# heng-hw/SpaCap3D

Measured on AMD Instinct MI355X. Metric: scenes/sec (40k pts, 256 proposals) fwd+bwd, higher is better.
Workload: dtype f32; 1 GPU; cfg2: synthetic ScanRefer-shaped scans, 40000 pts x (xyz+1 ch), 256 proposals, 8 scenes/GPU; full training step (SpaCapNet fwd + loss + bwd + grad all-reduce + Adam); global_batch=8, parallelism=dp1, hip_graph=True, fps_prefetch_side_stream=True, prefetch_as_graph=True, reserved_cus_forward=8, geometry_prefetch=True, deferred_weight_gradients=True, params=9290918, allreduce_bytes=35572416

## Files before the change

spacap3d_amd/csrc/sa_mlp.hip:

```cpp
#include <hipcub/hipcub.hpp>

#include <type_traits>

#include "common.hpp"
#include "mfma.hpp"
#include <atomic>

namespace {
using namespace spacap::mfma;

constexpr int TM = 64;
constexpr int TW = 32;
constexpr int NPART = 1024;


__device__ __forceinline__ long row_div(long r, long d) {
  if (((unsigned long long)r | (unsigned long long)d) >> 32) return r / d;
  return (long)((unsigned)r / (unsigned)d);
}

__device__ __forceinline__ f32x4 l1_row(f32x4 wx, f32x4 wy, f32x4 wz, f32x4 wf, f32x4 in, bool has_feat) {
  f32x4 z = wx * in[0] + wy * in[1] + wz * in[2];
  if (has_feat) z += wf * in[3];
  return z;
// ... 337 lines not shown
#pragma unroll
        for (int q = 0; q < KH; ++q)
#pragma unroll
          for (int u = 0; u < 4; ++u)
#pragma unroll
            for (int j = 0; j < NT; ++j)
              acc[mt][j] = MFMA16(wf[j][(h * KH + q) * 4 + u], bq[c & 1][q][u], acc[mt][j]);
        __builtin_amdgcn_sched_barrier(0);
        if (c + 2 < NCH) bload(c + 2);
      }
    }
#pragma unroll
    for (int mt = 0; mt < TMT / 16; ++mt)
#pragma unroll
      for (int j = 0; j < NT; ++j) {
        if (TAIL) {
          f32x4 v = acc[mt][j] + bv[j];
#pragma unroll
          for (int u = 0; u < 4; ++u) v[u] = fmaxf(v[u], 0.f);
          st4(&s_o[(mt * 16 + l15) * LDO + wc + 16 * j + 4 * lg], v);
        } else {
          st4(&s_o[(mt * 16 + l15) * LDO + wc + 16 * j + 4 * lg], acc[mt][j]);
          if (FULL || row0 + mt * 16 + l15 < R) {
            ssum[j] += acc[mt][j];
            ssq[j] += acc[mt][j] * acc[mt][j];
          }
        }
      }
    __syncthreads();
#pragma unroll
    for (int i = 0; i < NO; ++i) {
      const int row = or0 + i * OSTEP;
      if (FULL || row0 + row < R) st4(zout + (size_t)(row0 + row) * Cout + cbb + o4 * 4, ld4(&s_o[row * LDO + o4 * 4]));
    }
    if (TAIL) {
      f32x4 a3 = {0.f, 0.f, 0.f, 0.f};
#pragma unroll
      for (int ks = 0; ks < COB / 4; ++ks) a3 = MFMA16(wf3[TAIL ? ks : 0], s_o[(w * 16 + l15) * LDO + ks * 4 + lg], a3);
      const long row = row0 + w * 16 + l15;
      if (FULL || row < R) {
#pragma unroll
        for (int u = 0; u < 4; ++u)
          if (4 * lg + u < ta.NO3) ta.pred[(size_t)row * ta.NO3 + 4 * lg + u] = a3[u] + ta.b3[4 * lg + u];
      }
    }
  };
  const long nfull = R / TMT;
  bool pending = false;
  if ((long)blockIdx.x < nfull) fetch(blockIdx.x);
  for (long t = blockIdx.x; t < nfull; t += gridDim.x) {
    tile(t, std::true_type{}, pending);
    pending = true;
  }
  asm volatile("s_waitcnt vmcnt(0)" ::: "memory");
#pragma unroll
  for (int i = 0; i < NV; ++i) asm volatile("" ::"v"(pre[i]));
  if (nfull < ntiles && (long)blockIdx.x == nfull % gridDim.x) {
    fetch(nfull);
    tile(nfull, std::false_type{}, false);
  }
  if (TAIL) return;
#pragma unroll
  for (int j = 0; j < NT; ++j)
#pragma unroll
    for (int u = 0; u < 4; ++u) {
      float a = ssum[j][u], q = ssq[j][u];
#pragma unroll
      for (int o = 1; o < 16; o <<= 1) a += __shfl_xor(a, o), q += __shfl_xor(q, o);
      if (l15 == 0) {
        const int c = cb + 16 * j + 4 * lg + u;
        part[((size_t)blockIdx.x * 2 + 0) * Cout + c] = (double)a;
        part[((size_t)blockIdx.x * 2 + 1) * Cout + c] = (double)q;
        for (int pr = blockIdx.x + gridDim.x; pr < NPART; pr += gridDim.x)
          part[((size_t)pr * 2 + 0) * Cout + c] = 0.0, part[((size_t)pr * 2 + 1) * Cout + c] = 0.0;
      }
    }
}

using f32x16 = float __attribute__((ext_vector_type(16)));
#define MFMA_BF16(a, b, c) __builtin_amdgcn_mfma_f32_32x32x16_bf16((a), (b), (c), 0, 0, 0)

#include "sa_bf3.inc"
#include "sa_bf3_dgrad.inc"
#include "sa_l3bwd.inc"

__global__ __launch_bounds__(256) void sa_pool_fwd_kernel(const float *__restrict__ z, const float *__restrict__ st,
                                                          long G, int S, int C, float *__restrict__ out,
                                                          uint8_t *__restrict__ arg) {
  const int C4 = C / 4;
  const long i = (long)blockIdx.x * 256 + threadIdx.x;
  if (i >= G * C4) return;
  const long g = i / C4;
  const int c4 = (int)(i % C4);
  f32x4 mean, sc, be;
#pragma unroll
  for (int u = 0; u < 4; ++u) {
    const float *s = st + (size_t)(c4 * 4 + u) * 4;
    mean[u] = s[0], sc[u] = s[2], be[u] = s[3];
  }
  f32x4 best = {-1.f, -1.f, -1.f, -1.f};
  int bi[4] = {0, 0, 0, 0};
  const float *p = z + ((size_t)g * S) * C + c4 * 4;
#pragma unroll 4
  for (int s = 0; s < S; ++s, p += C) {
    const f32x4 v = ld4(p);
#pragma unroll
    for (int u = 0; u < 4; ++u) {
      const float a = fmaxf((v[u] - mean[u]) * sc[u] + be[u], 0.f);
      if (a > best[u]) best[u] = a, bi[u] = s;
    }
  }
  st4(out + (size_t)g * C + c4 * 4, best);
  *reinterpret_cast<uchar4 *>(arg + (size_t)g * C + c4 * 4) =
      make_uchar4((unsigned char)bi[0], (unsigned char)bi[1], (unsigned char)bi[2], (unsigned char)bi[3]);
}

__global__ __launch_bounds__(256) void sa_pool_bwd_kernel(const float *__restrict__ dout, const float *__restrict__ out,
                                                          const uint8_t *__restrict__ arg, const float *__restrict__ z,
                                                          const float *__restrict__ zmax, const float *__restrict__ st, long G,
                                                          int S, int C, float *__restrict__ dym, double *__restrict__ part) {
  __shared__ float s_red[2][256];
  const int tid = threadIdx.x;
  const int c = tid % C;
  const int gs = tid / C, GP = 256 / C;
  const float mean = st[c * 4], istd = st[c * 4 + 1];
  const bool from_max = zmax && (st[c * 4 + 2] != 0.f || !z);
  float s1 = 0.f, s2 = 0.f;
  for (long g = (long)blockIdx.x * GP + gs; g < G; g += (long)gridDim.x * GP) {
    const size_t o = (size_t)g * C + c;
    const float dy = out[o] > 0.f ? dout[o] : 0.f;
    dym[o] = dy;
    const float zz = from_max ? zmax[o] : z[((size_t)g * S + arg[o]) * C + c];
    s1 += dy;
    s2 += dy * ((zz - mean) * istd);
  }
  s_red[0][tid] = s1, s_red[1][tid] = s2;
  __syncthreads();
  if (tid < C) {
    double a = 0.0, b = 0.0;
    for (int i = 0; i < GP; ++i) a += (double)s_red[0][i * C + tid], b += (double)s_red[1][i * C + tid];
    part[((size_t)blockIdx.x * 2 + 0) * C + tid] = a;
    part[((size_t)blockIdx.x * 2 + 1) * C + tid] = b;
  }
}

template <bool POOLED>
__device__ __forceinline__ f32x4 load_dz(const float *__restrict__ dy, const uint8_t *__restrict__ arg, int S,
                                         const float *__restrict__ zk, long grow, int CK, int c0, f32x4 g, f32x4 k0,
                                         f32x4 k1) {
  const f32x4 z = ld4(zk + (size_t)grow * CK + c0);
  f32x4 d;
  if (POOLED) {
    const int lgS = (S & (S - 1)) == 0 ? __builtin_ctz((unsigned)S) : -1;
    const long grp = lgS >= 0 ? (grow >> lgS) : grow / S;
    const int s = (int)(grow - grp * S);
    const f32x4 dm = ld4(dy + (size_t)grp * CK + c0);
    const uchar4 a = *reinterpret_cast<const uchar4 *>(arg + (size_t)grp * CK + c0);
    d[0] = a.x == s ? dm[0] : 0.f;
    d[1] = a.y == s ? dm[1] : 0.f;
    d[2] = a.z == s ? dm[2] : 0.f;
    d[3] = a.w == s ? dm[3] : 0.f;
  } else {
    d = ld4(dy + (size_t)grow * CK + c0);
  }
  return g * d + k0 - k1 * z;
}

struct L1Args {
  const float *feat, *xyz, *new_xyz;
  const int32_t *idx;
  float rdiv;
  int Np, N, S;
  float *part;
  const float *rel4;
  L1In li;
  float *partW;
};

template <int CK, int NT, bool POOLED, bool PREFETCH, bool ALIAS, bool L1 = false, bool WG = false>
__global__ __launch_bounds__(256) __attribute__((amdgpu_waves_per_eu(L1 ? 2 : 1))) void sa_dgrad_kernel(const float *__restrict__ dy, const uint8_t *__restrict__ arg, int S,
                                                       const float *__restrict__ zk, const float *__restrict__ coef,
                                                       const float *__restrict__ Wk, int CP, const float *__restrict__ zp,
                                                       const float *__restrict__ st_p, long R, float *__restrict__ dyp,
                                                       double *__restrict__ part, const L1Args L = L1Args{}) {
  constexpr int LD = CK + 4, KS = CK / 4, C4 = CK / 4, NV = TM * C4 / 256, RSTEP = 256 / C4;
  constexpr int COB = 64 * NT, LDO = COB + 4, O4 = COB / 4, NO = TM * O4 / 256, OSTEP = 256 / O4;
  constexpr bool DENSE_PF = PREFETCH && !POOLED;
  extern __shared__ __attribute__((aligned(16))) float smem[];
  float *s_a = smem;
  float *s_o = ALIAS ? smem : smem + TM * LD;
  const int tid = threadIdx.x, lane = tid & 63, w = tid >> 6, l15 = lane & 15, lg = lane >> 4;
  const int cbb = blockIdx.y * COB, wc = w * 16 * NT, cb = cbb + wc;
  float wf[NT][KS];
#pragma unroll
  for (int j = 0; j < NT; ++j)
#pragma unroll
    for (int ks = 0; ks < KS; ++ks) wf[j][ks] = Wk[(size_t)(ks * 4 + lg) * CP + cb + 16 * j + l15];
  const int c4 = tid % C4, r0 = tid / C4, o4 = tid % O4, or0 = tid / O4;
  f32x4 g, k0, k1, pm, pi, ps, pb;
#pragma unroll
  for (int u = 0; u < 4; ++u) {
    const float *s = coef + (size_t)(c4 * 4 + u) * 4;
    g[u] = s[0], k0[u] = s[1], k1[u] = s[2];
    const float *q = st_p + (size_t)(cbb + o4 * 4 + u) * 4;
    pm[u] = q[0], pi[u] = q[1], ps[u] = q[2], pb[u] = q[3];
  }
  f32x4 s1 = {0.f, 0.f, 0.f, 0.f}, s2 = {0.f, 0.f, 0.f, 0.f};
  const int lgS = (S > 0 && (S & (S - 1)) == 0) ? __builtin_ctz((unsigned)S) : -1;
  const long ntiles = (R + TM - 1) / TM, nfull = R / TM;
  float *s_rel = smem + (ALIAS ? TM * LD : TM * LD + TM * LDO);
  f32x4 q1[L1 ? 4 : 1], q3[L1 ? 4 : 1], q2 = {0.f, 0.f, 0.f, 0.f};
  f32x4 l1x = {0.f, 0.f, 0.f, 0.f}, l1y = l1x, l1z = l1x, l1f = l1x;
  if (L1 && L.rel4) l1_weights(L.li, cbb + o4 * 4, l1x, l1y, l1z, l1f);
  if (L1) {
#pragma unroll
    for (int u = 0; u < 4; ++u) q1[u] = q3[u] = f32x4{0.f, 0.f, 0.f, 0.f};
  }
  static_assert(!WG || (L1 && !ALIAS && CK == 64 && NT == 1), "fused weight gradient: 64 x 64 first-layer instance only");
  f32x4 accw[WG ? 4 : 1];
#pragma unroll
  for (int n = 0; n < (WG ? 4 : 1); ++n) accw[n] = f32x4{0.f, 0.f, 0.f, 0.f};
  f32x4 pz[PREFETCH ? NV : 1], pd[DENSE_PF ? NV : 1];
  auto fetch = [&](long t) {
#pragma unroll
    for (int i = 0; i < NV; ++i) {
      long grow = t * TM + r0 + i * RSTEP;
      grow = grow < R ? grow : R - 1;
      const float *src = zk + (size_t)grow * CK + c4 * 4;
      asm volatile("global_load_dwordx4 %0, %1, off" : "=&v"(pz[i]) : "v"(src) : "memory");
      if (DENSE_PF) {
        const float *sd = dy + (size_t)grow * CK + c4 * 4;
        asm volatile("global_load_dwordx4 %0, %1, off" : "=&v"(pd[i]) : "v"(sd) : "memory");
      }
    }
  };
  auto tile = [&](long t, auto full, bool stores_pending) {
    constexpr bool FULL = decltype(full)::value;
    const long row0 = t * TM;
    if (PREFETCH) {
      if (stores_pending && !L1) asm volatile("s_waitcnt vmcnt(%0)" ::"n"(NO) : "memory");
      else asm volatile("s_waitcnt vmcnt(0)" ::: "memory");
#pragma unroll
      for (int i = 0; i < NV; ++i) {
        asm volatile("" : "+v"(pz[i]));
        if (DENSE_PF) asm volatile("" : "+v"(pd[i]));
      }
    }
#pragma unroll
    for (int i = 0; i < NV; ++i) {
      const int row = r0 + i * RSTEP;
      const long grow = row0 + row;
      f32x4 a = {0.f, 0.f, 0.f, 0.f};
      if (FULL || grow < R) {
        const f32x4 z = PREFETCH ? pz[i] : ld4(zk + (size_t)grow * CK + c4 * 4);
        f32x4 d;
        if (POOLED) {
          const long grp = lgS >= 0 ? (grow >> lgS) : grow / S;
          const int sidx = (int)(grow - grp * S);
          const f32x4 dm = ld4(dy + (size_t)grp * CK + c4 * 4);
          const uchar4 am = *reinterpret_cast<const uchar4 *>(arg + (size_t)grp * CK + c4 * 4);
          d[0] = am.x == sidx ? dm[0] : 0.f;
          d[1] = am.y == sidx ? dm[1] : 0.f;
          d[2] = am.z == sidx ? dm[2] : 0.f;
          d[3] = am.w == sidx ? dm[3] : 0.f;
        } else {
          d = DENSE_PF ? pd[i] : ld4(dy + (size_t)grow * CK + c4 * 4);
        }
        a = g * d + k0 - k1 * z;
      }
      st4(&s_a[row * LD + c4 * 4], a);
    }
    if (L1 && tid < TM) {
      f32x4 in = {0.f, 0.f, 0.f, 0.f};
      const long grow = row0 + tid;
      if ((FULL || grow < R) && L.rel4) {
        in = ld4(L.rel4 + (size_t)grow * 4);
      } else if (FULL || grow < R) {
        const long b = row_div(grow, (long)L.N * L.S), gi = row_div(grow, L.S);
        const int p = L.idx[grow];
        const float *q = L.xyz + ((size_t)b * L.Np + p) * 3, *c = L.new_xyz + (size_t)gi * 3;
        in[0] = (q[0] - c[0]) / L.rdiv, in[1] = (q[1] - c[1]) / L.rdiv, in[2] = (q[2] - c[2]) / L.rdiv;
        if (L.feat) in[3] = L.feat[(size_t)b * L.Np + p];
      }
      st4(&s_rel[tid * 4], in);
      q2 += in;
    }
    __syncthreads();
    if (PREFETCH && FULL) fetch(t + gridDim.x);
    f32x4 acc[TM / 16][NT];
#pragma unroll
    for (int mt = 0; mt < TM / 16; ++mt)
#pragma unroll
      for (int j = 0; j < NT; ++j) acc[mt][j] = f32x4{0.f, 0.f, 0.f, 0.f};
    {
#pragma unroll
      for (int ks = 0; ks < KS; ++ks) {
#pragma unroll
        for (int mt = 0; mt < TM / 16; ++mt) {
          const float b = s_a[(mt * 16 + l15) * LD + ks * 4 + lg];
#pragma unroll
          for (int j = 0; j < NT; ++j) acc[mt][j] = MFMA16(wf[j][ks], b, acc[mt][j]);
        }
      }
    }
    if (ALIAS) __syncthreads();
#pragma unroll
    for (int mt = 0; mt < TM / 16; ++mt)
#pragma unroll
      for (int j = 0; j < NT; ++j) st4(&s_o[(mt * 16 + l15) * LDO + wc + 16 * j + 4 * lg], acc[mt][j]);
    __syncthreads();
#pragma unroll
    for (int i = 0; i < NO; ++i) {
      const int row = or0 + i * OSTEP;
      if (FULL || row0 + row < R) {
        const size_t o = (size_t)(row0 + row) * CP + cbb + o4 * 4;
        const f32x4 da = ld4(&s_o[row * LDO + o4 * 4]);
        f32x4 z;
        if (L1 && L.rel4) z = l1_row(l1x, l1y, l1z, l1f, ld4(&s_rel[row * 4]), L.li.has_feat != 0);
        else z = ld4(zp + o);
        f32x4 d;
#pragma unroll
        for (int u = 0; u < 4; ++u) {
          const float pre = (z[u] - pm[u]) * ps[u] + pb[u];
          d[u] = pre > 0.f ? da[u] : 0.f;
          s1[u] += d[u];
          s2[u] += d[u] * ((z[u] - pm[u]) * pi[u]);
        }
        if (L1) {
          const f32x4 in = ld4(&s_rel[row * 4]);
#pragma unroll
          for (int u = 0; u < 4; ++u) {
            q1[u] += in * d[u];
            q3[u] += in * z[u];
          }
        } else {
          st4(dyp + o, d);
        }
        if (WG) {
          f32x4 ap;
#pragma unroll
          for (int u = 0; u < 4; ++u) ap[u] = fmaxf((z[u] - pm[u]) * ps[u] + pb[u], 0.f);
          st4(&s_o[row * LDO + o4 * 4], ap);
        }
      } else if (WG) {
        st4(&s_o[row * LDO + o4 * 4], f32x4{0.f, 0.f, 0.f, 0.f});
      }
    }
    if (WG) {
      __syncthreads();
#pragma unroll
      for (int ks = 0; ks < TM / 4; ++ks) {
        const float af = s_a[(ks * 4 + lg) * LD + 16 * w + l15];
#pragma unroll
        for (int n = 0; n < 4; ++n) accw[n] = MFMA16(af, s_o[(ks * 4 + lg) * LDO + 16 * n + l15], accw[n]);
      }
      __syncthreads();
    }
    if (ALIAS) __syncthreads();
  };
  bool pending = false;
  if (PREFETCH && (long)blockIdx.x < nfull) fetch(blockIdx.x);
  for (long t = blockIdx.x; t < nfull; t += gridDim.x) {
    tile(t, std::true_type{}, pending);
    pending = true;
  }
  if (PREFETCH) {
    asm volatile("s_waitcnt vmcnt(0)" ::: "memory");
#pragma unroll
    for (int i = 0; i < NV; ++i) {
      asm volatile("" ::"v"(pz[i]));
      if (DENSE_PF) asm volatile("" ::"v"(pd[i]));
    }
  }
  if (nfull < ntiles && (long)blockIdx.x == nfull % gridDim.x) {
    if (PREFETCH) {
      fetch(nfull);
    }
    tile(nfull, std::false_type{}, false);
  }
  __syncthreads();
  float *s_red = smem;
  st4(&s_red[(0 * OSTEP + or0) * COB + o4 * 4], s1);
  st4(&s_red[(1 * OSTEP + or0) * COB + o4 * 4], s2);
  __syncthreads();
  if (tid < 2 * COB) {
    const int k = tid / COB, c = tid % COB;
    float a = 0.f;
    for (int i = 0; i < OSTEP; ++i) a += s_red[(k * OSTEP + i) * COB + c];
    part[((size_t)blockIdx.x * 2 + k) * CP + cbb + c] = (double)a;
    for (int pr = blockIdx.x + gridDim.x; pr < NPART; pr += gridDim.x) part[((size_t)pr * 2 + k) * CP + cbb + c] = 0.0;
  }
  if (WG) {
    float *o = L.partW + (size_t)blockIdx.x * CK * COB;
#pragma unroll
    for (int n = 0; n < 4; ++n)
#pragma unroll
      for (int u = 0; u < 4; ++u) o[(size_t)(16 * w + 4 * lg + u) * COB + 16 * n + l15] = accw[n][u];
  }
  if (L1) {
    __syncthreads();
    float *s_q = smem;
#pragma unroll
    for (int u = 0; u < 4; ++u) {
      st4(&s_q[((or0 * COB) + o4 * 4 + u) * 8], q1[u]);
      st4(&s_q[((or0 * COB) + o4 * 4 + u) * 8 + 4], q3[u]);
    }
    __syncthreads();
    float *out = L.part + (size_t)blockIdx.x * (COB * 8 + 4);
    for (int e = tid; e < COB * 8; e += 256) {
      float a = 0.f;
      for (int i = 0; i < OSTEP; ++i) a += s_q[i * COB * 8 + e];
      out[e] = a;
    }
    __syncthreads();
    if (tid < TM) st4(&s_q[tid * 4], q2);
    __syncthreads();
    if (tid < 4) {
      float a = 0.f;
      for (int i = 0; i < TM; ++i) a += s_q[i * 4 + tid];
      out[COB * 8 + tid] = a;
    }
    for (int pr = blockIdx.x + gridDim.x; pr < NPART; pr += gridDim.x)
      for (int e = tid; e < COB * 8 + 4; e += 256) L.part[(size_t)pr * (COB * 8 + 4) + e] = 0.f;
  }
}

template <int CKB, int CP, bool POOLED>
__global__ __launch_bounds__(256) void sa_wgrad_kernel(const float *__restrict__ dy, const uint8_t *__restrict__ arg, int S,
                                                       const float *__restrict__ zk, const float *__restrict__ coef, int CK,
                                                       const float *__restrict__ zp, const float *__restrict__ st_p, long R,
                                                       float *__restrict__ partW, L1In li = L1In{nullptr, 0, 0}) {
// ... 420 lines not shown
    static const int res = resident_blocks(sa_wgrad_kernel<CKB, CPV, PV>, 0);   \
    return res;                                                                 \
  }
  if (pooled && CK % 128 == 0 && CP == 64) WR(128, 64, true)
  if (pooled && CK % 128 == 0 && CP == 128) WR(128, 128, true)
  if (!pooled && CK == 64 && CP == 64) WR(64, 64, false)
  if (!pooled && CK == 128 && CP == 128) WR(128, 128, false)
#undef WR
  return 512;
}
}
extern "C" int spacap_sa_wgrad_slabs(long R, int CK, int CP, int pooled) {
  const int gy = CK >= 128 ? CK / 128 : 1;
  long n = bwd_resident(wgrad_resident(CK, CP, pooled != 0)) / gy, cap = (16L << 20) / ((long)CK * CP), tiles = (R + TW - 1) / TW;
  if (n > cap) n = cap;
  if (n > tiles) n = tiles;
  return (int)(n < 1 ? 1 : n);
}

extern "C" int spacap_sa_mlp_supported(int C1, int C2, int C3) {
  const bool sa1 = (C1 == 64 && C2 == 64 && C3 == 128);
  const bool big = (C1 == 128 && C2 == 128 && (C3 == 128 || C3 == 256));
  return (sa1 || big) ? 1 : 0;
}

extern "C" int spacap_sa_l1_fwd_f32(const float *Y, const float *feat, const float *xyz, const float *new_xyz,
                                    const int32_t *idx, const float *W1, int ldw, float rdiv, int B, int Np, int N,
                                    int S, int C1, float *z1, double *part, spacap_stream_t stream) {
  const char *what = "spacap_sa_l1_fwd_f32";
  SPACAP_REQUIRE(B >= 1 && Np >= 1 && N >= 1 && S >= 1 && S <= 255, "%s: bad sizes", what);
  SPACAP_REQUIRE(C1 == 64 || C1 == 128, "%s: C1=%d unsupported", what, C1);
  SPACAP_REQUIRE(xyz && new_xyz && idx && W1 && z1 && part && ldw >= (feat ? 4 : 3) && rdiv > 0.f, "%s: bad arguments", what);
  const long R = (long)B * N * S;
  hipStream_t s = spacap::as_stream(stream);
  if (C1 == 64)
    hipLaunchKernelGGL((sa_l1_fwd_kernel<64>), dim3(NPART), dim3(256), 0, s, Y, feat, xyz, new_xyz, idx, W1, ldw, rdiv, Np, N, S, R, z1, part);
  else
    hipLaunchKernelGGL((sa_l1_fwd_kernel<128>), dim3(NPART), dim3(256), 0, s, Y, feat, xyz, new_xyz, idx, W1, ldw, rdiv, Np, N, S, R, z1, part);
  SPACAP_CHECK_LAUNCH(what);
  return SPACAP_OK;
}

extern "C" int spacap_sa_l1_stats_f32(const float *feat, const float *xyz, const float *new_xyz, const int32_t *idx, const float *W1,
                                      int ldw, float rdiv, int B, int Np, int N, int S, int C1, float *rel4, double *part,
                                      spacap_stream_t stream) {
  const char *what = "spacap_sa_l1_stats_f32";
  SPACAP_REQUIRE(B >= 1 && Np >= 1 && N >= 1 && S >= 1 && S <= 255, "%s: bad sizes", what);
  SPACAP_REQUIRE(C1 == 64, "%s: C1=%d unsupported", what, C1);
  SPACAP_REQUIRE(xyz && new_xyz && idx && W1 && rel4 && part && ldw >= (feat ? 4 : 3) && rdiv > 0.f, "%s: bad arguments", what);
  const long R = (long)B * N * S;
  hipLaunchKernelGGL((sa_l1_fwd_kernel<64>), dim3(NPART), dim3(256), 0, spacap::as_stream(stream), (const float *)nullptr, feat, xyz,
                     new_xyz, idx, W1, ldw, rdiv, Np, N, S, R, (float *)nullptr, part, rel4);
  SPACAP_CHECK_LAUNCH(what);
  return SPACAP_OK;
}

extern "C" int spacap_sa_l1_moments_f32(const float *feat, const float *xyz, const float *new_xyz, const int32_t *idx, float rdiv, int B,
                                        int Np, int N, int S, float *rel4, double *mom, spacap_stream_t stream) {
  const char *what = "spacap_sa_l1_moments_f32";
  SPACAP_REQUIRE(B >= 1 && Np >= 1 && N >= 1 && S >= 1 && S <= 255, "%s: bad sizes", what);
  SPACAP_REQUIRE(xyz && new_xyz && idx && rel4 && mom && rdiv > 0.f && (reinterpret_cast<uintptr_t>(rel4) & 15) == 0, "%s: bad arguments", what);
  const long R = (long)B * N * S;
  hipLaunchKernelGGL(sa_l1_moments_kernel, dim3(NPART), dim3(256), 0, spacap::as_stream(stream), feat, xyz, new_xyz, idx, rdiv, Np, N, S, R,
                     rel4, mom);
  SPACAP_CHECK_LAUNCH(what);
  return SPACAP_OK;
}

extern "C" int spacap_sa_l1_moments_finalize_f32(const double *mom, const float *W1, int ldw, int has_feat, int C1, long count, float eps,
                                                 float momentum, const float *gamma, const float *beta, float *running_mean,
                                                 float *running_var, float *stats, spacap_stream_t stream) {
  const char *what = "spacap_sa_l1_moments_finalize_f32";
  SPACAP_REQUIRE(mom && W1 && gamma && beta && stats && C1 >= 1 && C1 <= 1024 && count >= 1 && ldw >= (has_feat ? 4 : 3), "%s: bad arguments", what);
  hipLaunchKernelGGL(sa_l1_moments_finalize_kernel, dim3(1), dim3(1024), 0, spacap::as_stream(stream), mom, NPART, W1, ldw, has_feat, C1,
                     (double)count, eps, momentum, gamma, beta, running_mean, running_var, stats);
  SPACAP_CHECK_LAUNCH(what);
  return SPACAP_OK;
}

extern "C" int spacap_sa_mid_fwd_l1in_f32(const float *rel4, const float *W1, int ldw, int has_feat, const float *st_in, const float *W,
                                          long R, float *zout, double *part, spacap_stream_t stream) {
  const char *what = "spacap_sa_mid_fwd_l1in_f32";
  SPACAP_REQUIRE(rel4 && W1 && st_in && W && zout && part && R >= 1 && ldw >= (has_feat ? 4 : 3), "%s: bad arguments", what);
  const size_t lds = (size_t)TM * ((64 + 8) + (64 + 4)) * sizeof(float);
  const long tiles = (R + TM - 1) / TM;
  static const int res = resident_blocks(sa_mid_fwd_kernel<64, 1, false>, lds);
  hipLaunchKernelGGL((sa_mid_fwd_kernel<64, 1, false>), dim3(grid_rows(res, 1, tiles), 1), dim3(256), lds, spacap::as_stream(stream),
                     rel4, st_in, W, 64, R, zout, part, TailArgs{}, L1In{W1, ldw, has_feat});
  SPACAP_CHECK_LAUNCH(what);
  return SPACAP_OK;
}

extern "C" int spacap_sa_wgrad_l1in_f32(const float *dy, const float *zk, const float *coef, const float *rel4, const float *W1, int ldw,
                                        int has_feat, const float *st_p, long R, float *partW, spacap_stream_t stream) {
  const char *what = "spacap_sa_wgrad_l1in_f32";
  SPACAP_REQUIRE(dy && zk && coef && rel4 && W1 && st_p && partW && R >= 1 && ldw >= (has_feat ? 4 : 3), "%s: bad arguments", what);
  const int nslab = spacap_sa_wgrad_slabs(R, 64, 64, 0);
  hipLaunchKernelGGL((sa_wgrad_kernel<64, 64, false>), dim3(nslab, 1), dim3(256), 0, spacap::as_stream(stream), dy, (const uint8_t *)nullptr,
                     0, zk, coef, 64, rel4, st_p, R, partW, L1In{W1, ldw, has_feat});
  SPACAP_CHECK_LAUNCH(what);
  return SPACAP_OK;
}

extern "C" int spacap_sa_bn_finalize_f32(const double *part, int C, long count, float eps, float momentum,
                                         const float *gamma, const float *beta, float *running_mean,
                                         float *running_var, float *stats, spacap_stream_t stream) {
  const char *what = "spacap_sa_bn_finalize_f32";
  SPACAP_REQUIRE(part && gamma && beta && stats && C >= 1 && count >= 1, "%s: bad arguments", what);
  hipLaunchKernelGGL(sa_bn_finalize_kernel, dim3((C + 7) / 8), dim3(1024), 0, spacap::as_stream(stream), part, NPART, C,
                     (double)count, eps, momentum, gamma, beta, running_mean, running_var, stats);
  SPACAP_CHECK_LAUNCH(what);
  return SPACAP_OK;
}

extern "C" int spacap_sa_bwd_finalize_f32(const double *part, int C, long count, const float *stats, float *coef,
                                          float *dgamma, float *dbeta, spacap_stream_t stream) {
  const char *what = "spacap_sa_bwd_finalize_f32";
  SPACAP_REQUIRE(part && stats && coef && dgamma && dbeta && C >= 1 && count >= 1, "%s: bad arguments", what);
  hipLaunchKernelGGL(sa_bwd_finalize_kernel, dim3((C + 7) / 8), dim3(1024), 0, spacap::as_stream(stream), part, NPART, C,
                     (double)count, stats, coef, dgamma, dbeta);
  SPACAP_CHECK_LAUNCH(what);
  return SPACAP_OK;
}

extern "C" int spacap_sa_mid_fwd_f32(const float *zin, const float *st_in, const float *W, long R, int Cin, int Cout,
                                     float *zout, double *part, spacap_stream_t stream) {
  const char *what = "spacap_sa_mid_fwd_f32";
  SPACAP_REQUIRE(zin && st_in && W && zout && part && R >= 1, "%s: bad arguments", what);
  hipStream_t s = spacap::as_stream(stream);
  const int nt = (Cin == 64 && Cout == 64) ? 1 : 2;
  if (!f32_mfma_only() && (Cin == 64 || Cin == 128) && Cout % 128 == 0) {
    static const int cus = resident_blocks(sa_mid_fwd_bf3s_kernel<128, 1>, 100 * 1024);
    const size_t ldss = bf3s_lds_bytes(Cin);
    const long wtiles = (R + 31) / 32;
    const int gy = Cout / 128;
    long gx = (cus - reserved_cus()) / gy;
    gx = gx > NPART ? NPART : gx;
    gx = gx > (wtiles + 7) / 8 ? (wtiles + 7) / 8 : gx;
    if (Cin == 64)
      hipLaunchKernelGGL((sa_mid_fwd_bf3s_kernel<64, 1>), dim3((unsigned)gx, gy), dim3(512), ldss, s, zin, st_in, W, Cout, R, zout,
                         part, PoolArgs{});
    else
      hipLaunchKernelGGL((sa_mid_fwd_bf3s_kernel<128, 1>), dim3((unsigned)gx, gy), dim3(512), ldss, s, zin, st_in, W, Cout, R, zout,
                         part, PoolArgs{});
    SPACAP_CHECK_LAUNCH(what);
    return SPACAP_OK;
  }
  const size_t lds = (size_t)TM * ((Cin + 8) + (64 * nt + 4)) * sizeof(float);
  const long tiles = (R + TM - 1) / TM;
#define MF(CI, NTV, GY)                                                                                              \
  {                                                                                                                  \
    static const int res = resident_blocks(sa_mid_fwd_kernel<CI, NTV, false>, lds);                                  \
    hipLaunchKernelGGL((sa_mid_fwd_kernel<CI, NTV, false>), dim3(grid_rows(res, GY, tiles), GY), dim3(256), lds, s,  \
                       zin, st_in, W, Cout, R, zout, part, TailArgs{});                                              \
  }
  if (Cin == 64 && Cout == 64) MF(64, 1, 1)
  else if (Cin == 64 && Cout % 128 == 0) MF(64, 2, Cout / 128)
  else if (Cin == 128 && Cout % 128 == 0) MF(128, 2, Cout / 128)
  else
    SPACAP_REQUIRE(false, "%s: (Cin=%d, Cout=%d) unsupported", what, Cin, Cout);
#undef MF
  SPACAP_CHECK_LAUNCH(what);
  return SPACAP_OK;
}

__global__ __launch_bounds__(256) void sa_pool_finalize_kernel(const float *__restrict__ cand_v, const uint8_t *__restrict__ cand_i,
                                                               const float *__restrict__ st, const float *__restrict__ gamma,
                                                               long G, int S, int C, float *__restrict__ out,
// ... 183 lines not shown
}

extern "C" int spacap_sa_dgrad_f32(const float *dy, const uint8_t *arg, int S, const float *zk, const float *coef,
                                   const float *Wk, const float *zp, const float *st_p, long R, int CK, int CP,
                                   float *dyp, double *part, spacap_stream_t stream) {
  const char *what = "spacap_sa_dgrad_f32";
  SPACAP_REQUIRE(dy && zk && coef && Wk && zp && st_p && dyp && part && R >= 1, "%s: bad arguments", what);
  SPACAP_REQUIRE(!arg || (S >= 1 && R % S == 0), "%s: bad S", what);
  hipStream_t s = spacap::as_stream(stream);
  if (!f32_mfma_only() && (CK == 128 || CK == 256) && CP % 64 == 0 && R >= 49152) {
    static const int cus = resident_blocks(sa_mid_fwd_bf3s_kernel<128, 1>, 100 * 1024);
    const size_t ldsd = bf3s_dgrad_lds_bytes(CK);
    const long wtiles = (R + 31) / 32;
    const int gy = CP / 64;
    long gx = bwd_resident(cus) / gy;
    gx = gx > NPART ? NPART : gx;
    gx = gx > (wtiles + 7) / 8 ? (wtiles + 7) / 8 : gx;
#define DS(CKV, PV)                                                                                                   \
  hipLaunchKernelGGL((sa_dgrad_bf3s_kernel<CKV, PV>), dim3((unsigned)gx, gy), dim3(512), ldsd, s, dy, arg, S, zk, coef, Wk, CP, zp, \
                     st_p, R, dyp, part)
    if (CK == 128) { if (arg) DS(128, true); else DS(128, false); }
    else { if (arg) DS(256, true); else DS(256, false); }
#undef DS
    SPACAP_CHECK_LAUNCH(what);
    return SPACAP_OK;
  }
#define DG(CKV, NTV, PV, PF, AL, GY)                                                                                 \
  {                                                                                                                  \
    const size_t lds = (size_t)TM * ((CKV + 4) + ((AL) ? 0 : (64 * NTV + 4))) * sizeof(float);                       \
    if (lds > 65536)                                                                                                 \
      SPACAP_CHECK_HIP(hipFuncSetAttribute(reinterpret_cast<const void *>(&sa_dgrad_kernel<CKV, NTV, PV, PF, AL>),   \
                                           hipFuncAttributeMaxDynamicSharedMemorySize, (int)lds), what);            \
    static const int res = resident_blocks(sa_dgrad_kernel<CKV, NTV, PV, PF, AL>, lds);                              \
    hipLaunchKernelGGL((sa_dgrad_kernel<CKV, NTV, PV, PF, AL>), dim3(grid_rows(bwd_resident(res), GY, (R + TM - 1) / TM), GY), \
                       dim3(256), lds, s, dy, arg, S, zk, coef, Wk, CP, zp, st_p, R, dyp, part);                      \
  }
  if (arg && CK == 128 && CP == 64) DG(128, 1, true, true, false, 1)
  else if (arg && CK == 256 && CP == 128) DG(256, 1, true, false, true, 2)
  else if (arg && CK == 128 && CP == 128) DG(128, 2, true, true, false, 1)
  else if (!arg && CK == 64 && CP == 64) DG(64, 1, false, true, false, 1)
  else if (!arg && CK == 128 && CP == 128) DG(128, 2, false, true, false, 1)
  else SPACAP_REQUIRE(false, "%s: (CK=%d, CP=%d, pooled=%d) unsupported", what, CK, CP, arg ? 1 : 0);
#undef DG
  SPACAP_CHECK_LAUNCH(what);
  return SPACAP_OK;
}

extern "C" int spacap_sa_dgrad_l1_f32(const float *dy, const float *zk, const float *coef, const float *Wk, const float *zp,
                                      const float *st_p, const float *feat, const float *xyz, const float *new_xyz,
                                      const int32_t *idx, float rdiv, int B, int Np, int N, int S, int CK, int CP,
                                      double *part, float *part_l1, spacap_stream_t stream) {
  const char *what = "spacap_sa_dgrad_l1_f32";
  SPACAP_REQUIRE(dy && zk && coef && Wk && zp && st_p && xyz && new_xyz && idx && part && part_l1 && rdiv > 0.f,
                 "%s: bad arguments", what);
  SPACAP_REQUIRE(CK == 64 && CP == 64, "%s: (CK=%d, CP=%d) unsupported", what, CK, CP);
  const long R = (long)B * N * S;
  hipStream_t s = spacap::as_stream(stream);
  const size_t lds = (size_t)TM * ((64 + 4) + (64 + 4) + 4) * sizeof(float);
  static const int res = resident_blocks(sa_dgrad_kernel<64, 1, false, true, false, true>, lds);
  L1Args L{feat, xyz, new_xyz, idx, rdiv, Np, N, S, part_l1, nullptr, L1In{nullptr, 0, 0}, nullptr};
  hipLaunchKernelGGL((sa_dgrad_kernel<64, 1, false, true, false, true>), dim3(grid_rows(bwd_resident(res), 1, (R + TM - 1) / TM), 1),
                     dim3(256), lds, s, dy, (const uint8_t *)nullptr, 0, zk, coef, Wk, CP, zp, st_p, R, (float *)nullptr, part, L);
  SPACAP_CHECK_LAUNCH(what);
  return SPACAP_OK;
}

extern "C" int spacap_sa_dgrad_l1in_f32(const float *dy, const float *zk, const float *coef, const float *Wk, const float *rel4,
                                        const float *W1, int ldw, int has_feat, const float *st_p, int B, int N, int S, double *part,
                                        float *part_l1, spacap_stream_t stream) {
  const char *what = "spacap_sa_dgrad_l1in_f32";
  SPACAP_REQUIRE(dy && zk && coef && Wk && rel4 && W1 && st_p && part && part_l1 && ldw >= (has_feat ? 4 : 3), "%s: bad arguments", what);
  const long R = (long)B * N * S;
  const size_t lds = (size_t)TM * ((64 + 4) + (64 + 4) + 4) * sizeof(float);
  static const int res = resident_blocks(sa_dgrad_kernel<64, 1, false, true, false, true>, lds);
  L1Args L{nullptr, nullptr, nullptr, nullptr, 1.f, 1, N, S, part_l1, rel4, L1In{W1, ldw, has_feat}, nullptr};
  hipLaunchKernelGGL((sa_dgrad_kernel<64, 1, false, true, false, true>), dim3(grid_rows(bwd_resident(res), 1, (R + TM - 1) / TM), 1),
                     dim3(256), lds, spacap::as_stream(stream), dy, (const uint8_t *)nullptr, 0, zk, coef, Wk, 64, (const float *)nullptr,
                     st_p, R, (float *)nullptr, part, L);
  SPACAP_CHECK_LAUNCH(what);
  return SPACAP_OK;
}

namespace {
int dgrad_wgrad_l1in_grid(long R) {
  const size_t lds = (size_t)TM * ((64 + 4) + (64 + 4) + 4) * sizeof(float);
  static const int res = resident_blocks(sa_dgrad_kernel<64, 1, false, true, false, true, true>, lds);
  return grid_rows(bwd_resident(res), 1, (R + TM - 1) / TM);
}
}
extern "C" int spacap_sa_dgrad_wgrad_l1in_slabs(long R) { return R >= 1 ? dgrad_wgrad_l1in_grid(R) : 0; }
extern "C" int spacap_sa_dgrad_wgrad_l1in_f32(const float *dy, const float *zk, const float *coef, const float *Wk, const float *rel4,
                                              const float *W1, int ldw, int has_feat, const float *st_p, int B, int N, int S,
                                              double *part, float *part_l1, float *partW, spacap_stream_t stream) {
  const char *what = "spacap_sa_dgrad_wgrad_l1in_f32";
  SPACAP_REQUIRE(dy && zk && coef && Wk && rel4 && W1 && st_p && part && part_l1 && partW && ldw >= (has_feat ? 4 : 3), "%s: bad arguments", what);
  const long R = (long)B * N * S;
  const size_t lds = (size_t)TM * ((64 + 4) + (64 + 4) + 4) * sizeof(float);
  L1Args L{nullptr, nullptr, nullptr, nullptr, 1.f, 1, N, S, part_l1, rel4, L1In{W1, ldw, has_feat}, partW};
  hipLaunchKernelGGL((sa_dgrad_kernel<64, 1, false, true, false, true, true>), dim3(dgrad_wgrad_l1in_grid(R), 1), dim3(256), lds,
                     spacap::as_stream(stream), dy, (const uint8_t *)nullptr, 0, zk, coef, Wk, 64, (const float *)nullptr, st_p, R,
                     (float *)nullptr, part, L);
  SPACAP_CHECK_LAUNCH(what);
  return SPACAP_OK;
}

namespace {
__global__ __launch_bounds__(256) void sa_l1_dw_kernel(const float *__restrict__ part_l1, int nparts, const float *__restrict__ coef,
                                                       int C1, int ldw, float *__restrict__ dW1) {
  __shared__ double s_lane[12][17];
  __shared__ double s_sum[12];
  const int c = blockIdx.x, tid = threadIdx.x, sidx = tid >> 4, l = tid & 15;
  const int n = C1 * 8 + 4;
  if (sidx < 12) {
    const int e = sidx < 8 ? c * 8 + sidx : C1 * 8 + (sidx - 8);
    double a0 = 0.0, a1 = 0.0, a2 = 0.0, a3 = 0.0;
    int p = l;
    for (; p + 48 < nparts; p += 64) {
      a0 += (double)part_l1[(size_t)p * n + e];
      a1 += (double)part_l1[(size_t)(p + 16) * n + e];
      a2 += (double)part_l1[(size_t)(p + 32) * n + e];
      a3 += (double)part_l1[(size_t)(p + 48) * n + e];
    }
    for (; p < nparts; p += 16) a0 += (double)part_l1[(size_t)p * n + e];
    s_lane[sidx][l] = (a0 + a1) + (a2 + a3);
  }
  __syncthreads();
  if (tid < 12) {
    double a = 0.0;
    for (int i = 0; i < 16; ++i) a += s_lane[tid][i];
    s_sum[tid] = a;
  }
  __syncthreads();
  if (tid < ldw) {
    const double g = coef[c * 4 + 0], k0 = coef[c * 4 + 1], k1 = coef[c * 4 + 2];
    dW1[c * ldw + tid] = (float)(g * s_sum[tid] + k0 * s_sum[8 + tid] - k1 * s_sum[4 + tid]);
  }
}
}
extern "C" int spacap_sa_l1_dw_f32(const float *part_l1, int nparts, const float *coef, int C1, int ldw, float *dW1,
                                   spacap_stream_t stream) {
  const char *what = "spacap_sa_l1_dw_f32";
  SPACAP_REQUIRE(part_l1 && coef && dW1 && nparts >= 1 && C1 >= 1 && C1 <= 512 && ldw >= 1 && ldw <= 4, "%s: bad arguments", what);
  hipLaunchKernelGGL(sa_l1_dw_kernel, dim3(C1), dim3(256), 0, spacap::as_stream(stream), part_l1, nparts, coef, C1, ldw, dW1);
  SPACAP_CHECK_LAUNCH(what);
  return SPACAP_OK;
}

extern "C" int spacap_sa_wgrad_f32(const float *dy, const uint8_t *arg, int S, const float *zk, const float *coef,
                                   const float *zp, const float *st_p, long R, int CK, int CP, float *partW,
                                   spacap_stream_t stream) {
  const char *what = "spacap_sa_wgrad_f32";
  SPACAP_REQUIRE(dy && zk && coef && zp && st_p && partW && R >= 1, "%s: bad arguments", what);
  SPACAP_REQUIRE(!arg || (S >= 1 && R % S == 0), "%s: bad S", what);
  hipStream_t s = spacap::as_stream(stream);
  const int nslab = spacap_sa_wgrad_slabs(R, CK, CP, arg ? 1 : 0);
#define WG(CKB, CPV, PV) \
  hipLaunchKernelGGL((sa_wgrad_kernel<CKB, CPV, PV>), dim3(nslab, CK / CKB), dim3(256), 0, s, dy, arg, S, zk, coef, CK, zp, st_p, R, partW)
  if (arg && CK % 128 == 0 && CP == 64) WG(128, 64, true);
  else if (arg && CK % 128 == 0 && CP == 128) WG(128, 128, true);
  else if (!arg && CK == 64 && CP == 64) WG(64, 64, false);
  else if (!arg && CK == 128 && CP == 128) WG(128, 128, false);
  else SPACAP_REQUIRE(false, "%s: (CK=%d, CP=%d, pooled=%d) unsupported", what, CK, CP, arg ? 1 : 0);
#undef WG
  SPACAP_CHECK_LAUNCH(what);
  return SPACAP_OK;
}

extern "C" int spacap_sa_l1_bwd_f32(float *dy1, const float *z1, const float *coef, const float *feat, const float *xyz,
                                    const float *new_xyz, const int32_t *idx, const float *W1, int ldw, float rdiv, int B,
                                    int Np, int N, int S, int C1, float *partW, float *drel, int write_dz,
                                    spacap_stream_t stream) {
  const char *what = "spacap_sa_l1_bwd_f32";
  SPACAP_REQUIRE(dy1 && z1 && coef && xyz && new_xyz && idx && W1 && partW && rdiv > 0.f, "%s: bad arguments", what);
  SPACAP_REQUIRE(C1 == 64 || C1 == 128, "%s: C1=%d unsupported", what, C1);
  const long R = (long)B * N * S;
  hipStream_t s = spacap::as_stream(stream);
  if (C1 == 64)
    hipLaunchKernelGGL((sa_l1_bwd_kernel<64>), dim3(NPART), dim3(256), 0, s, dy1, z1, coef, feat, xyz, new_xyz, idx, W1, ldw, rdiv, Np, N, S, R, partW, drel, write_dz);
  else
    hipLaunchKernelGGL((sa_l1_bwd_kernel<128>), dim3(NPART), dim3(256), 0, s, dy1, z1, coef, feat, xyz, new_xyz, idx, W1, ldw, rdiv, Np, N, S, R, partW, drel, write_dz);
  SPACAP_CHECK_LAUNCH(what);
// ... 92 lines not shown
```

Baseline: 1164 scenes/s.

## Use split-bf16 MFMA for first-layer SA forward and fused dgrad/wgrad

Adds a split-bf16 (three-term) MFMA forward kernel for the 64x64 SA layer fed by the layer-1 input. It also adds a BF3/WGB path in the fused dgrad+weight-gradient kernel, so activations and gradients are staged as bf16 hi/mid/lo images in LDS and multiplied with bf16 MFMA instead of f32 MFMA. The aim is to replace slower f32 matrix instructions with faster bf16 ones while keeping near-f32 accuracy through the 3-way split. This costs extra split and pack work, a larger or different LDS footprint (which may change occupancy), and small numerical differences.

```diff
diff --git a/spacap3d_amd/csrc/sa_bf3_l1in.inc b/spacap3d_amd/csrc/sa_bf3_l1in.inc
--- /dev/null
+++ b/spacap3d_amd/csrc/sa_bf3_l1in.inc
@@ -0,0 +1,119 @@
+__device__ __forceinline__ void wave_lds_fence() {
+  __builtin_amdgcn_fence(__ATOMIC_RELEASE, "wavefront");
+  __builtin_amdgcn_wave_barrier();
+  __builtin_amdgcn_fence(__ATOMIC_ACQUIRE, "wavefront");
+}
+
+__global__ __launch_bounds__(256) __attribute__((amdgpu_waves_per_eu(2))) void sa_l1in_fwd_bf3_kernel(
+    const float *__restrict__ rel4, const L1In li, const float *__restrict__ st_in, const float *__restrict__ W, long R,
+    float *__restrict__ zout, double *__restrict__ part) {
+  constexpr int C = 64, TR = 16, LDA = C + 16, IMG = TR * LDA, LDO = C + 4, NW = 4;
+  __shared__ __attribute__((aligned(16))) __bf16 s_img[NW][3][IMG];
+  __shared__ __attribute__((aligned(16))) float s_out[NW][TR * LDO];
+  __shared__ float s_red[NW][2][C];
+  const int tid = threadIdx.x, lane = tid & 63, w = tid >> 6, l15 = lane & 15, lg = lane >> 4;
+  __bf16 *img = &s_img[w][0][0];
+  float *so = &s_out[w][0];
+  bf16x8 wA[4][2][3];
+#pragma unroll
+  for (int n = 0; n < 4; ++n)
+#pragma unroll
+    for (int s = 0; s < 2; ++s) {
+      const float *wp = W + (size_t)(16 * n + l15) * C + 32 * s + 8 * lg;
+      split8(ld4(wp), ld4(wp + 4), wA[n][s]);
+    }
+  const int c4 = l15, rr = lg;
+  f32x4 mean, sc, be;
+#pragma unroll
+  for (int u = 0; u < 4; ++u) {
+    const float *s = st_in + (size_t)(c4 * 4 + u) * 4;
+    mean[u] = s[0], sc[u] = s[2], be[u] = s[3];
+  }
+  f32x4 l1x, l1y, l1z, l1f;
+  l1_weights(li, c4 * 4, l1x, l1y, l1z, l1f);
+  f32x4 ssum[4], ssq[4];
+#pragma unroll
+  for (int n = 0; n < 4; ++n) ssum[n] = ssq[n] = f32x4{0.f, 0.f, 0.f, 0.f};
+  const long ntiles = (R + TR - 1) / TR;
+  const long gw = (long)blockIdx.x * NW + w, GW = (long)gridDim.x * NW;
+  f32x4 pre[4];
+  auto fetch = [&](long t) {
+#pragma unroll
+    for (int i = 0; i < 4; ++i) {
+      long grow = t * TR + rr + 4 * i;
+      grow = grow < R ? grow : R - 1;
+      pre[i] = ld4(rel4 + (size_t)grow * 4);
+    }
+  };
+  if (gw < ntiles) fetch(gw);
+  for (long t = gw; t < ntiles; t += GW) {
+    const long row0 = t * TR;
+    const bool full = row0 + TR <= R;
+#pragma unroll
+    for (int i = 0; i < 4; ++i) {
+      const int row = rr + 4 * i;
+      const f32x4 zv = l1_row(l1x, l1y, l1z, l1f, pre[i], li.has_feat != 0);
+      f32x4 a;
+#pragma unroll
+      for (int u = 0; u < 4; ++u) a[u] = fmaxf((zv[u] - mean[u]) * sc[u] + be[u], 0.f);
+      if (!full && row0 + row >= R) a = f32x4{0.f, 0.f, 0.f, 0.f};
+      bf16x4 p0, p1, p2;
+      split4(a, p0, p1, p2);
+      const int o = row * LDA + c4 * 4;
+      *reinterpret_cast<bf16x4 *>(img + o) = p0;
+      *reinterpret_cast<bf16x4 *>(img + IMG + o) = p1;
+      *reinterpret_cast<bf16x4 *>(img + 2 * IMG + o) = p2;
+    }
+    fetch(t + GW < ntiles ? t + GW : t);
+    wave_lds_fence();
+    bf16x8 b[2][3];
+#pragma unroll
+    for (int s = 0; s < 2; ++s)
+#pragma unroll
+      for (int q = 0; q < 3; ++q) b[s][q] = *reinterpret_cast<const bf16x8 *>(img + q * IMG + l15 * LDA + 32 * s + 8 * lg);
+    f32x4 acc[4];
+#pragma unroll
+    for (int n = 0; n < 4; ++n) acc[n] = f32x4{0.f, 0.f, 0.f, 0.f};
+#pragma unroll
+    for (int s = 0; s < 2; ++s)
+#pragma unroll
+      for (int q = 0; q < 6; ++q)
+#pragma unroll
+        for (int n = 0; n < 4; ++n) acc[n] = MFMA_B(wA[n][s][PA[q]], b[s][PB[q]], acc[n]);
+    const bool mine = full || row0 + l15 < R;
+#pragma unroll
+    for (int n = 0; n < 4; ++n) {
+      if (mine) {
+        ssum[n] += acc[n];
+        ssq[n] += acc[n] * acc[n];
+      }
+      st4(so + l15 * LDO + 16 * n + 4 * lg, acc[n]);
+    }
+    wave_lds_fence();
+#pragma unroll
+    for (int i = 0; i < 4; ++i) {
+      const int row = rr + 4 * i;
+      if (full || row0 + row < R) st4(zout + (size_t)(row0 + row) * C + c4 * 4, ld4(so + row * LDO + c4 * 4));
+    }
+    wave_lds_fence();
+  }
+#pragma unroll
+  for (int n = 0; n < 4; ++n)
+#pragma unroll
+    for (int u = 0; u < 4; ++u) {
+      float a = ssum[n][u], q = ssq[n][u];
+#pragma unroll
+      for (int o = 1; o < 16; o <<= 1) a += __shfl_xor(a, o), q += __shfl_xor(q, o);
+      if (l15 == 0) s_red[w][0][16 * n + 4 * lg + u] = a, s_red[w][1][16 * n + 4 * lg + u] = q;
+    }
+  __syncthreads();
+  if (tid < 2 * C) {
+    const int k = tid / C, c = tid % C;
+    double a = 0.0;
+#pragma unroll
+    for (int ww = 0; ww < NW; ++ww) a += (double)s_red[ww][k][c];
+    part[((size_t)blockIdx.x * 2 + k) * C + c] = a;
+    for (int pr = blockIdx.x + gridDim.x; pr < NPART; pr += gridDim.x)
+      part[((size_t)pr * 2 + k) * C + c] = 0.0;
+  }
+}
diff --git a/spacap3d_amd/csrc/sa_mlp.hip b/spacap3d_amd/csrc/sa_mlp.hip
--- a/spacap3d_amd/csrc/sa_mlp.hip
+++ b/spacap3d_amd/csrc/sa_mlp.hip
@@ -443,6 +443,7 @@
 
 #include "sa_bf3.inc"
 #include "sa_bf3_dgrad.inc"
+#include "sa_bf3_l1in.inc"
 #include "sa_l3bwd.inc"
 
 __global__ __launch_bounds__(256) void sa_pool_fwd_kernel(const float *__restrict__ z, const float *__restrict__ st,
@@ -538,7 +539,7 @@
   float *partW;
 };
 
-template <int CK, int NT, bool POOLED, bool PREFETCH, bool ALIAS, bool L1 = false, bool WG = false>
+template <int CK, int NT, bool POOLED, bool PREFETCH, bool ALIAS, bool L1 = false, bool WG = false, bool BF3 = false, bool WGB = false>
 __global__ __launch_bounds__(256) __attribute__((amdgpu_waves_per_eu(L1 ? 2 : 1))) void sa_dgrad_kernel(const float *__restrict__ dy, const uint8_t *__restrict__ arg, int S,
                                                        const float *__restrict__ zk, const float *__restrict__ coef,
                                                        const float *__restrict__ Wk, int CP, const float *__restrict__ zp,
@@ -547,16 +548,33 @@
   constexpr int LD = CK + 4, KS = CK / 4, C4 = CK / 4, NV = TM * C4 / 256, RSTEP = 256 / C4;
   constexpr int COB = 64 * NT, LDO = COB + 4, O4 = COB / 4, NO = TM * O4 / 256, OSTEP = 256 / O4;
   constexpr bool DENSE_PF = PREFETCH && !POOLED;
+  static_assert((!BF3 || WG) && (!WGB || BF3), "split-bf16 products: the fused 64 x 64 first-layer instance only");
+  constexpr int LDB = CK + 16, IMGB = TM * LDB;
+  constexpr int AF = (BF3 && WGB) ? 0 : TM * LD;
   extern __shared__ __attribute__((aligned(16))) float smem[];
   float *s_a = smem;
-  float *s_o = ALIAS ? smem : smem + TM * LD;
+  float *s_o = ALIAS ? smem : smem + AF;
   const int tid = threadIdx.x, lane = tid & 63, w = tid >> 6, l15 = lane & 15, lg = lane >> 4;
   const int cbb = blockIdx.y * COB, wc = w * 16 * NT, cb = cbb + wc;
-  float wf[NT][KS];
-#pragma unroll
-  for (int j = 0; j < NT; ++j)
-#pragma unroll
-    for (int ks = 0; ks < KS; ++ks) wf[j][ks] = Wk[(size_t)(ks * 4 + lg) * CP + cb + 16 * j + l15];
+  float wf[BF3 ? 1 : NT][BF3 ? 1 : KS];
+  bf16x8 wB[BF3 ? CK / 32 : 1][3];
+  if constexpr (BF3) {
+#pragma unroll
+    for (int s = 0; s < CK / 32; ++s) {
+      f32x4 lo, hi;
+#pragma unroll
+      for (int e = 0; e < 4; ++e) {
+        lo[e] = Wk[(size_t)(32 * s + 8 * lg + e) * CP + cb + l15];
+        hi[e] = Wk[(size_t)(32 * s + 8 * lg + 4 + e) * CP + cb + l15];
+      }
+      split8(lo, hi, wB[s]);
+    }
+  } else {
+#pragma unroll
+    for (int j = 0; j < NT; ++j)
+#pragma unroll
+      for (int ks = 0; ks < KS; ++ks) wf[j][ks] = Wk[(size_t)(ks * 4 + lg) * CP + cb + 16 * j + l15];
+  }
   const int c4 = tid % C4, r0 = tid / C4, o4 = tid % O4, or0 = tid / O4;
   f32x4 g, k0, k1, pm, pi, ps, pb;
 #pragma unroll
@@ -569,7 +587,9 @@
   f32x4 s1 = {0.f, 0.f, 0.f, 0.f}, s2 = {0.f, 0.f, 0.f, 0.f};
   const int lgS = (S > 0 && (S & (S - 1)) == 0) ? __builtin_ctz((unsigned)S) : -1;
   const long ntiles = (R + TM - 1) / TM, nfull = R / TM;
-  float *s_rel = smem + (ALIAS ? TM * LD : TM * LD + TM * LDO);
+  float *s_rel = smem + (ALIAS ? TM * LD : AF + TM * LDO);
+  __bf16 *s_dzb = reinterpret_cast<__bf16 *>(s_rel + TM * 4);
+  __bf16 *s_apb = s_dzb + 3 * IMGB;
   f32x4 q1[L1 ? 4 : 1], q3[L1 ? 4 : 1], q2 = {0.f, 0.f, 0.f, 0.f};
   f32x4 l1x = {0.f, 0.f, 0.f, 0.f}, l1y = l1x, l1z = l1x, l1f = l1x;
   if (L1 && L.rel4) l1_weights(L.li, cbb + o4 * 4, l1x, l1y, l1z, l1f);
@@ -629,7 +649,15 @@
         }
         a = g * d + k0 - k1 * z;
       }
-      st4(&s_a[row * LD + c4 * 4], a);
+      if (!(BF3 && WGB)) st4(&s_a[row * LD + c4 * 4], a);
+      if constexpr (BF3) {
+        bf16x4 p0, p1, p2;
+        split4(a, p0, p1, p2);
+        const int o = row * LDB + c4 * 4;
+        *reinterpret_cast<bf16x4 *>(&s_dzb[o]) = p0;
+        *reinterpret_cast<bf16x4 *>(&s_dzb[IMGB + o]) = p1;
+        *reinterpret_cast<bf16x4 *>(&s_dzb[2 * IMGB + o]) = p2;
+      }
     }
     if (L1 && tid < TM) {
       f32x4 in = {0.f, 0.f, 0.f, 0.f};
@@ -653,7 +681,25 @@
     for (int mt = 0; mt < TM / 16; ++mt)
 #pragma unroll
       for (int j = 0; j < NT; ++j) acc[mt][j] = f32x4{0.f, 0.f, 0.f, 0.f};
-    {
+    if constexpr (BF3) {
+      bf16x8 b[2][CK / 32][3];
+      auto bload = [&](int mt) {
+#pragma unroll
+        for (int s = 0; s < CK / 32; ++s)
+#pragma unroll
+          for (int q = 0; q < 3; ++q)
+            b[mt & 1][s][q] = *reinterpret_cast<const bf16x8 *>(&s_dzb[q * IMGB + (mt * 16 + l15) * LDB + 32 * s + 8 * lg]);
+      };
+      bload(0);
+#pragma unroll
+      for (int mt = 0; mt < TM / 16; ++mt) {
+        __builtin_amdgcn_sched_barrier(0);
+        if (mt + 1 < TM / 16) bload(mt + 1);
+#pragma unroll
+        for (int s = 0; s < CK / 32; ++s) acc[mt][0] = mfma6(wB[s], b[mt & 1][s], acc[mt][0]);
+      }
+      __builtin_amdgcn_sched_barrier(0);
+    } else {
 #pragma unroll
       for (int ks = 0; ks < KS; ++ks) {
 #pragma unroll
@@ -701,13 +747,42 @@
           f32x4 ap;
 #pragma unroll
           for (int u = 0; u < 4; ++u) ap[u] = fmaxf((z[u] - pm[u]) * ps[u] + pb[u], 0.f);
-          st4(&s_o[row * LDO + o4 * 4], ap);
+          if constexpr (WGB) {
+            bf16x4 p0, p1, p2;
+            split4(ap, p0, p1, p2);
+            const int ob = row * LDB + o4 * 4;
+            *reinterpret_cast<bf16x4 *>(&s_apb[ob]) = p0;
+            *reinterpret_cast<bf16x4 *>(&s_apb[IMGB + ob]) = p1;
+            *reinterpret_cast<bf16x4 *>(&s_apb[2 * IMGB + ob]) = p2;
+          } else {
+            st4(&s_o[row * LDO + o4 * 4], ap);
+          }
         }
+      } else if (WGB) {
+        const bf16x4 zero = {(__bf16)0.f, (__bf16)0.f, (__bf16)0.f, (__bf16)0.f};
+#pragma unroll
+        for (int q = 0; q < 3; ++q) *reinterpret_cast<bf16x4 *>(&s_apb[q * IMGB + row * LDB + o4 * 4]) = zero;
       } else if (WG) {
         st4(&s_o[row * LDO + o4 * 4], f32x4{0.f, 0.f, 0.f, 0.f});
       }
     }
-    if (WG) {
+    if constexpr (WGB) {
+      __syncthreads();
+#pragma unroll
+      for (int s = 0; s < TM / 32; ++s) {
+        bf16x8 a[3];
+#pragma unroll
+        for (int q = 0; q < 3; ++q) a[q] = tr_frag<LDB>(s_dzb + q * IMGB + 32 * s * LDB, 16 * w, lane);
+#pragma unroll
+        for (int n = 0; n < 4; ++n) {
+          bf16x8 b[3];
+#pragma unroll
+          for (int q = 0; q < 3; ++q) b[q] = tr_frag<LDB>(s_apb + q * IMGB + 32 * s * LDB, 16 * n, lane);
+          accw[n] = mfma6(a, b, accw[n]);
+        }
+      }
+      __syncthreads();
+    } else if (WG) {
       __syncthreads();
 #pragma unroll
       for (int ks = 0; ks < TM / 4; ++ks) {
@@ -1294,8 +1369,15 @@
                                           long R, float *zout, double *part, spacap_stream_t stream) {
   const char *what = "spacap_sa_mid_fwd_l1in_f32";
   SPACAP_REQUIRE(rel4 && W1 && st_in && W && zout && part && R >= 1 && ldw >= (has_feat ? 4 : 3), "%s: bad arguments", what);
+  const long tiles = (R + TM - 1) / TM;
+  if (!f32_mfma_only()) {
+    static const int res = resident_blocks(sa_l1in_fwd_bf3_kernel, 0);
+    hipLaunchKernelGGL(sa_l1in_fwd_bf3_kernel, dim3(grid_rows(res, 1, tiles), 1), dim3(256), 0, spacap::as_stream(stream), rel4,
+                       L1In{W1, ldw, has_feat}, st_in, W, R, zout, part);
+    SPACAP_CHECK_LAUNCH(what);
+    return SPACAP_OK;
+  }
   const size_t lds = (size_t)TM * ((64 + 8) + (64 + 4)) * sizeof(float);
-  const long tiles = (R + TM - 1) / TM;
   static const int res = resident_blocks(sa_mid_fwd_kernel<64, 1, false>, lds);
   hipLaunchKernelGGL((sa_mid_fwd_kernel<64, 1, false>), dim3(grid_rows(res, 1, tiles), 1), dim3(256), lds, spacap::as_stream(stream),
                      rel4, st_in, W, 64, R, zout, part, TailArgs{}, L1In{W1, ldw, has_feat});
@@ -1645,9 +1727,22 @@
 }
 
 namespace {
+#ifndef SPACAP_L2_WGB
+#define SPACAP_L2_WGB 1
+#endif
+constexpr bool L2_WGB = SPACAP_L2_WGB != 0;
+constexpr size_t DWL_LDS_F32 = (size_t)TM * ((64 + 4) + (64 + 4) + 4) * sizeof(float);
+constexpr size_t DWL_LDS_BF3 = (size_t)TM * ((L2_WGB ? 0 : 64 + 4) + (64 + 4) + 4) * sizeof(float) + (size_t)(L2_WGB ? 2 : 1) * 3 * TM * (64 + 16) * 2;
 int dgrad_wgrad_l1in_grid(long R) {
-  const size_t lds = (size_t)TM * ((64 + 4) + (64 + 4) + 4) * sizeof(float);
-  static const int res = resident_blocks(sa_dgrad_kernel<64, 1, false, true, false, true, true>, lds);
+  if (!f32_mfma_only()) {
+    static unsigned long long lds_ok = 0;
+    if (spacap::allow_dynamic_lds(reinterpret_cast<const void *>(&sa_dgrad_kernel<64, 1, false, true, false, true, true, true, L2_WGB>),
+                                  (int)DWL_LDS_BF3, lds_ok) != hipSuccess)
+      (void)hipGetLastError();
+    static const int res = resident_blocks(sa_dgrad_kernel<64, 1, false, true, false, true, true, true, L2_WGB>, DWL_LDS_BF3);
+    return grid_rows(bwd_resident(res), 1, (R + TM - 1) / TM);
+  }
+  static const int res = resident_blocks(sa_dgrad_kernel<64, 1, false, true, false, true, true>, DWL_LDS_F32);
   return grid_rows(bwd_resident(res), 1, (R + TM - 1) / TM);
 }
 }
@@ -1658,8 +1753,14 @@
   const char *what = "spacap_sa_dgrad_wgrad_l1in_f32";
   SPACAP_REQUIRE(dy && zk && coef && Wk && rel4 && W1 && st_p && part && part_l1 && partW && ldw >= (has_feat ? 4 : 3), "%s: bad arguments", what);
   const long R = (long)B * N * S;
-  const size_t lds = (size_t)TM * ((64 + 4) + (64 + 4) + 4) * sizeof(float);
   L1Args L{nullptr, nullptr, nullptr, nullptr, 1.f, 1, N, S, part_l1, rel4, L1In{W1, ldw, has_feat}, partW};
+  if (!f32_mfma_only()) {
+    hipLaunchKernelGGL((sa_dgrad_kernel<64, 1, false, true, false, true, true, true, L2_WGB>), dim3(dgrad_wgrad_l1in_grid(R), 1), dim3(256), DWL_LDS_BF3, spacap::as_stream(stream), dy,
+                       (const uint8_t *)nullptr, 0, zk, coef, Wk, 64, (const float *)nullptr, st_p, R, (float *)nullptr, part, L);
+    SPACAP_CHECK_LAUNCH(what);
+    return SPACAP_OK;
+  }
+  const size_t lds = DWL_LDS_F32;
   hipLaunchKernelGGL((sa_dgrad_kernel<64, 1, false, true, false, true, true>), dim3(dgrad_wgrad_l1in_grid(R), 1), dim3(256), lds,
                      spacap::as_stream(stream), dy, (const uint8_t *)nullptr, 0, zk, coef, Wk, 64, (const float *)nullptr, st_p, R,
                      (float *)nullptr, part, L);
```

Result: no change. 1155 scenes/s (-0.7%).
